# antbern/gridmap-slam-robot

Measured on AMD Instinct MI355X. Metric: particle-scan evals/sec, higher is better.
Workload: dtype f64; 1 GPU; C3: 16384 particles/GPU x 720 beams (697 hits), 2048x2048 grid @ 0.02 m, full scan step (score+normalise+resample+ray-cast+likelihood rebuild; the rebuild is dirty-tile / factor-table-only: bit-identical results, likelihoodData on demand -- the reference's own every-cell rebuild is cpu_baseline.gpu_like_for_like_ms_per_step); particles_total=16384, particles_per_gpu=16384, beams=720, maps=1, maps_total=1, parallelism=single GPU, inputs=resident in HBM

## Files before the change

### gridmap_slam_robot_amd/csrc/gms_fused_kernels.hip

```cpp
#include "gms_map_kernels.hip"
#include "gms_pf_kernels.hip"
#include "gms_slam_kernels.hip"

#ifndef GMS_APPLY_BLOCKS_RIDING
#define GMS_APPLY_BLOCKS_RIDING 512
#endif

#ifndef RCF_RAYS
#define RCF_RAYS 4
#endif

template <bool LOGNORM>
__global__ void __launch_bounds__(256)
k_norm_raycast(GridDev g, const gms_beam *__restrict__ beams, int32_t B, uint32_t *__restrict__ cnt, int32_t *__restrict__ bbox,
               int32_t nw_max, uint32_t n_ray_blocks,
               const double *__restrict__ partials, int64_t nblk_global, double *__restrict__ w, const float *__restrict__ pose,
               int32_t n, int64_t offset, PackedParticle *__restrict__ packed, double *__restrict__ cum,
               double *__restrict__ chunk_tot, int64_t nchunks, double *__restrict__ p2, PfStatsDev *__restrict__ stats,
               uint32_t n_norm_blocks, double *__restrict__ logd, uint32_t *__restrict__ cnt_pend, const int32_t *__restrict__ bbox_pend,
               uint32_t n_near_blocks, const double *__restrict__ logw_lognorm, uint32_t *__restrict__ res_ticket,
               double *__restrict__ res_pre) {
    extern __shared__ __align__(16) unsigned char smem[];
    GMS_STAMP(GMS_STAMP_ROW(2, blockIdx.x), 0);
    if (blockIdx.x >= n_ray_blocks + n_norm_blocks) {
        apply_body(g, logd, cnt_pend, bbox_pend, nullptr, blockIdx.x - n_ray_blocks - n_norm_blocks, 0,
                   gridDim.x - n_ray_blocks - n_norm_blocks);
        GMS_STAMP(GMS_STAMP_ROW(2, blockIdx.x), 15);
        return;
    }
    if (blockIdx.x < n_ray_blocks) {
        __shared__ RedLds L;
        __shared__ float s_pose[3];
        const int cols[4] = { COL_SUM, COL_XW, COL_YW, COL_TW };
        double f[4];
        if (LOGNORM) {
            fold_lognorm<4>(partials, nblk_global, cols, f, L);
        } else {
            fold_sums<4>(partials, nblk_global, cols, f, L);
        }
        if (threadIdx.x == 0) {
            s_pose[0] = (float)(f[1] / f[0]);
            s_pose[1] = (float)(f[2] / f[0]);
            s_pose[2] = (float)(f[3] / f[0]);
        }
        __syncthreads();
        GMS_STAMP(GMS_STAMP_ROW(2, blockIdx.x), 1);
        if (blockIdx.x >= n_ray_blocks - n_near_blocks)
            raycast_near_body(g, beams, B, B, nullptr, 0, cnt, bbox, blockIdx.x - (n_ray_blocks - n_near_blocks), 0, smem, s_pose);
        else
            raycast_body<false, RCF_RAYS, 4>(g, beams, B, B, nullptr, 0, nullptr, cnt, bbox, nullptr, nullptr, 0, nullptr, nw_max, blockIdx.x, 0,
                                             smem, s_pose, n_near_blocks ? 1 : 0);
    } else {
        normalize_pack_body(partials, nblk_global, w, pose, n, offset, packed, cum, chunk_tot, nchunks, p2, stats,
                            blockIdx.x - n_ray_blocks, 0, LOGNORM ? logw_lognorm : (const double *)nullptr, res_ticket, n_norm_blocks,
                            res_pre, smem);
        GMS_STAMP(GMS_STAMP_ROW(2, blockIdx.x), 14);
    }
}

__global__ void __launch_bounds__(256)
k_partials_apply(double *__restrict__ w, double *__restrict__ logw, const float *__restrict__ pose, int32_t n, int64_t offset,
                 int64_t nblk_global, double *__restrict__ partials, const double *__restrict__ part, int32_t part_nseg,
                 GridDev g, double *__restrict__ logd, uint32_t *__restrict__ cnt, const int32_t *__restrict__ bbox,
                 int32_t *__restrict__ bbox_idle, PfStatsDev *__restrict__ lognorm_stats) {
    if (blockIdx.x < (uint32_t)nblk_global)
        partials_body(w, logw, pose, n, offset, nblk_global, partials, part, part_nseg, blockIdx.x, blockIdx.y, lognorm_stats);
    else
        apply_body(g, logd, cnt, bbox, bbox_idle, blockIdx.x - (uint32_t)nblk_global, blockIdx.y, gridDim.x - (uint32_t)nblk_global);
}

__global__ void __launch_bounds__(256)
k_partials_pack_apply(double *__restrict__ w, double *__restrict__ logw, const float *__restrict__ pose, int32_t n, int64_t offset,
                      int64_t nblk_global, double *__restrict__ partials, const double *__restrict__ part, int32_t part_nseg,
                      PackedParticle *__restrict__ packed_local, uint32_t n_local_blocks,
                      GridDev g, double *__restrict__ logd, uint32_t *__restrict__ cnt, const int32_t *__restrict__ bbox,
                      int32_t *__restrict__ bbox_idle) {
    if (blockIdx.x < n_local_blocks) {
        partials_body(w, logw, pose, n, offset, nblk_global, partials, part, part_nseg, (uint32_t)(offset / GMS_BLOCK) + blockIdx.x, 0);
        pack_raw_block(w, pose, n, blockIdx.x, packed_local);
    } else {
        apply_body(g, logd, cnt, bbox, bbox_idle, blockIdx.x - n_local_blocks, 0, gridDim.x - n_local_blocks);
    }
}

__global__ void __launch_bounds__(256)
k_raycast_norm_chunks(GridDev g, const gms_beam *__restrict__ beams, int32_t B, uint32_t *__restrict__ cnt, int32_t *__restrict__ bbox,
                      int32_t nw_max, uint32_t n_ray_blocks, uint32_t n_norm_blocks,
                      const double *__restrict__ partials, int64_t nblk_global, double *__restrict__ w, const float *__restrict__ pose,
                      int32_t n, int64_t offset, const PackedParticle *__restrict__ glob_raw, int64_t n_global, int64_t nchunks,
                      double *__restrict__ cum, double *__restrict__ chunk_tot, double *__restrict__ p2,
                      PfStatsDev *__restrict__ stats, uint32_t n_chunk_blocks, double *__restrict__ logd,
                      uint32_t *__restrict__ cnt_pend, const int32_t *__restrict__ bbox_pend, uint32_t n_near_blocks) {
    extern __shared__ __align__(16) unsigned char smem[];
    if (blockIdx.x >= n_ray_blocks + n_norm_blocks + n_chunk_blocks) {
        const uint32_t first = n_ray_blocks + n_norm_blocks + n_chunk_blocks;
        apply_body(g, logd, cnt_pend, bbox_pend, nullptr, blockIdx.x - first, 0, gridDim.x - first);
        return;
    }
    if (blockIdx.x < n_ray_blocks) {
        __shared__ RedLds L;
        __shared__ float s_pose[3];
        const int cols[4] = { COL_SUM, COL_XW, COL_YW, COL_TW };
        double f[4];
        fold_sums<4>(partials, nblk_global, cols, f, L);
        if (threadIdx.x == 0) {
            s_pose[0] = (float)(f[1] / f[0]);
            s_pose[1] = (float)(f[2] / f[0]);
            s_pose[2] = (float)(f[3] / f[0]);
        }
        __syncthreads();
        if (blockIdx.x >= n_ray_blocks - n_near_blocks)
            raycast_near_body(g, beams, B, B, nullptr, 0, cnt, bbox, blockIdx.x - (n_ray_blocks - n_near_blocks), 0, smem, s_pose);
        else
            raycast_body<false, RCF_RAYS, 4>(g, beams, B, B, nullptr, 0, nullptr, cnt, bbox, nullptr, nullptr, 0, nullptr, nw_max, blockIdx.x, 0,
                                             smem, s_pose, n_near_blocks ? 1 : 0);
    } else if (blockIdx.x < n_ray_blocks + n_norm_blocks) {
        normalize_own_body(partials, nblk_global, w, pose, n, offset, glob_raw, stats, blockIdx.x - n_ray_blocks);
    } else {
        chunk_sums_raw_body(glob_raw, n_global, nchunks, cum, chunk_tot, p2, nblk_global, partials,
                            blockIdx.x - n_ray_blocks - n_norm_blocks);
    }
}

template <int KH, int SPLIT>
__global__ void __launch_bounds__(256)
k_lik_resample(GridDev g, const double *__restrict__ logd, double *__restrict__ lik, double *__restrict__ fac, int64_t fac_stride,
               const double *__restrict__ taps_g, const int32_t *__restrict__ bbox, int32_t tiles_x, int32_t tiles_y,
               const uint32_t *__restrict__ cnt_pending, uint8_t *__restrict__ tile_state, uint32_t n_res_blocks,
               const PackedParticle *__restrict__ glob, int64_t n_global, int64_t nchunks, const double *__restrict__ cum,
               const double *__restrict__ chunk_off, const double *__restrict__ r01_maps, double r01, double fraction,
               int32_t n, int64_t offset,
               float *__restrict__ pose2, float *__restrict__ cs2, double *__restrict__ w2, int32_t *__restrict__ idx_out,
               const double *__restrict__ p2, int64_t nblk_global, PfStatsDev *__restrict__ stats, int32_t raw_weights,
               int32_t *__restrict__ bbox_clear, int32_t lik_mode, const double *__restrict__ res_pre) {
    extern __shared__ __align__(16) unsigned char smem[];
    GMS_STAMP(GMS_STAMP_ROW(3, blockIdx.x), 0);
    if (blockIdx.x == 0 && threadIdx.x < 4) bbox_clear[4 * blockIdx.y + threadIdx.x] = 0;
    if (blockIdx.x < n_res_blocks)
        resample_body(glob, n_global, nchunks, cum, chunk_off, r01_maps, r01, fraction, n, offset, pose2, cs2, w2, idx_out, p2,
                      nblk_global, stats, blockIdx.x, blockIdx.y, smem, raw_weights != 0, res_pre);
    else
        likelihood_body<KH, SPLIT>(g, logd, lik, fac, fac_stride, taps_g, bbox, 1, tiles_x, tiles_y, blockIdx.x - n_res_blocks,
                                   blockIdx.y, gridDim.x - n_res_blocks, smem, cnt_pending, tile_state, lik_mode);
    GMS_STAMP(GMS_STAMP_ROW(3, blockIdx.x), blockIdx.x < n_res_blocks ? 1 : 2);
}

__global__ void __launch_bounds__(256)
k_deskew_motion(const double *__restrict__ angle, const double *__restrict__ distance, const uint8_t *__restrict__ hit, int32_t length,
// ... 160 lines not shown
```

### gridmap_slam_robot_amd/csrc/gms_map_kernels.hip

```cpp
#include "gms_device.h"

__device__ __forceinline__ void bbox_decode(const int32_t *bb, int32_t W, int32_t H, int32_t &x0, int32_t &y0,
                                            int32_t &x1, int32_t &y1) {
    x0 = W - 1 - bb[0]; y0 = H - 1 - bb[1]; x1 = bb[2]; y1 = bb[3];
}


struct RayMeta {
    int32_t x0, y0, x_inc, y_inc, n_eff, hit;
    float sx, sy, measured;
    int32_t hx, hy;
};

#define RC_VALID 0x80000000u
#define RC_BOX_MARGIN 5

typedef __attribute__((address_space(3))) uint64_t gms_lds_u64;
typedef __attribute__((address_space(3))) uint32_t gms_lds_u32;
typedef __attribute__((address_space(3))) double gms_lds_f64;
__device__ __forceinline__ uint32_t lds_offset(const uint64_t *p) { return (uint32_t)(uintptr_t)(const gms_lds_u64 *)p; }
__device__ __forceinline__ void lds_publish_u64(uint64_t *p, uint64_t v) {
    asm volatile("ds_write_b64 %0, %1" : : "v"(lds_offset(p)), "v"(v) : "memory");
}
__device__ __forceinline__ void lds_poll_2xu64(const uint64_t *p0, const uint64_t *p1, uint64_t &a, uint64_t &c) {
    asm volatile("ds_read_b64 %0, %2\n\t"
                 "ds_read_b64 %1, %3\n\t"
                 "s_waitcnt lgkmcnt(0)"
                 : "=&v"(a), "=&v"(c) : "v"(lds_offset(p0)), "v"(lds_offset(p1)) : "memory");
}

__device__ __forceinline__ RayMeta ray_meta(const GridDev &g, const RayIn &ray, RayDev &r) {
    RayMeta mt;
    ray_init(r, ray.sx + 0.5f, ray.sy + 0.5f, ray.ex + 0.5f, ray.ey + 0.5f, g.extra);
    mt.x0 = r.x; mt.y0 = r.y; mt.x_inc = r.x_inc; mt.y_inc = r.y_inc;
    mt.sx = ray.sx; mt.sy = ray.sy; mt.measured = ray.measured; mt.hit = ray.hit;
    const bool inb0 = !(r.x < 0 || r.x >= g.W || r.y < 0 || r.y >= g.H);
    mt.n_eff = (inb0 && r.n > 0) ? min(r.n, g.W + g.H + 1) : 0;
    const int64_t ax = llabs((int64_t)j_d2i(floor((double)(ray.ex + 0.5f))) - (int64_t)r.x) + g.extra + RC_BOX_MARGIN;
    const int64_t ay = llabs((int64_t)j_d2i(floor((double)(ray.ey + 0.5f))) - (int64_t)r.y) + g.extra + RC_BOX_MARGIN;
    const int32_t moves = mt.n_eff > 0 ? mt.n_eff - 1 : 0;
    mt.hx = min(max(r.x + r.x_inc * (int32_t)min((int64_t)moves, ax), 0), g.W - 1);
    mt.hy = min(max(r.y + r.y_inc * (int32_t)min((int64_t)moves, ay), 0), g.H - 1);
    return mt;
}
__device__ __forceinline__ void ray_box(const GridDev &g, const RayMeta &mt, int32_t bb[4]) {
    if (mt.n_eff <= 0) { bb[0] = bb[1] = bb[2] = bb[3] = 0; return; }
    bb[0] = g.W - 1 - min(mt.x0, mt.hx); bb[1] = g.H - 1 - min(mt.y0, mt.hy);
    bb[2] = max(mt.x0, mt.hx) + 1;       bb[3] = max(mt.y0, mt.hy) + 1;
}
__device__ __forceinline__ void bbox_raise_wave(int32_t bb[4], int32_t lane, int32_t *__restrict__ bbox_map) {
#define GMS_STEP_(O) { _Pragma("unroll") for (int q = 0; q < 4; q++) bb[q] = max(bb[q], wave_xor<O>(bb[q])); }
    GMS_BUTTERFLY(GMS_STEP_)
#undef GMS_STEP_
    if (lane == 0 && bb[2] > 0)
        for (int q = 0; q < 4; q++) atomicMax(&bbox_map[q], bb[q]);
}

struct RayWalk {
    float err, ndx, dy;
    uint32_t ycount;
};
__device__ __forceinline__ RayWalk ray_walk_begin(const RayDev &r) {
    RayWalk k;
    k.err = r.error; k.ndx = -r.dx; k.dy = r.dy; k.ycount = 0;
    asm volatile("" : "+v"(k.ndx), "+v"(k.dy));
    return k;
}
__device__ __forceinline__ void ray_phase_a(RayWalk &k, int32_t w0, int32_t w1, uint64_t *__restrict__ slots, int32_t stride, int32_t slot) {
    float err = k.err;
    const float ndx = k.ndx, dy = k.dy;
    uint32_t ycount = k.ycount;
    for (int32_t w = w0; w < w1; ++w) {
        uint32_t word = 0;
        float t;
#define GMS_DDA_STEP "v_cmp_lt_f32_e32 vcc, 0, %0\n\tv_cndmask_b32_e32 %2, %3, %4, vcc\n\tv_add_f32_e32 %0, %0, %2\n\tv_addc_co_u32_e32 %1, vcc, %1, %1, vcc\n\t"
// ... 37 lines not shown
        const int32_t ny = (int32_t)(((uint32_t)(sl >> 32) & ~RC_VALID) + __popc((uint32_t)sl & ((1u << j) - 1u)));
        const int32_t nx = k - ny;
        const int32_t cx = mt.x0 + mt.x_inc * nx, cy = mt.y0 + mt.y_inc * ny;
        valid = !(cx < 0 || cx >= g.W || cy < 0 || cy >= g.H);
        if (valid) {
            const float d = cell_distance(mt.sx, mt.sy, cx, cy);
            const int32_t cls = sensor_class(d, mt.measured, mt.hit, g.half_tol);
            if (TRACE) {
                if (k < cap) {
                    const size_t o = (size_t)b * cap + k;
                    if (t_cells) { t_cells[2 * o] = cx; t_cells[2 * o + 1] = cy; }
                    if (t_cls) t_cls[o] = (uint8_t)cls;
                }
            } else if (cls != 1) {
                const uint32_t inc = cls == 0 ? 1u : 0x10000u;
                const uint32_t ux = (uint32_t)(cx - tile.x0), uy = (uint32_t)(cy - tile.y0);
                if (ux < (uint32_t)tile.w && uy < (uint32_t)tile.h) {
                    const uint32_t ci = uy * (uint32_t)tile.w + ux;
                    __hip_atomic_fetch_add((gms_lds_u32 *)(tile.cells) + (ci >> 1), (cls == 0 ? 1u : 0x100u) << ((ci & 1u) << 4),
                                           __ATOMIC_RELAXED, __HIP_MEMORY_SCOPE_WORKGROUP);
                } else {
                    atomicAdd(&mcnt[(size_t)cy * g.W + cx], inc);
                    if (__builtin_expect(cx < min(mt.x0, mt.hx) || cx > max(mt.x0, mt.hx) || cy < min(mt.y0, mt.hy) || cy > max(mt.y0, mt.hy), 0)) {
                        atomicMax(&bbox_map[0], g.W - 1 - cx); atomicMax(&bbox_map[1], g.H - 1 - cy);
                        atomicMax(&bbox_map[2], cx + 1);       atomicMax(&bbox_map[3], cy + 1);
                    }
                }
            }
        }
    }
    return __popcll(__ballot(valid));
}

template <bool TRACE, int RC_RAYS, int NWAVES = RC_RAYS>
__device__ __forceinline__ void
raycast_body(const GridDev &g, const gms_beam *__restrict__ beams, int32_t B, int32_t beam_stride,
             const float *__restrict__ poses, int32_t pose_stride, const RayIn *__restrict__ single,
             uint32_t *__restrict__ cnt, int32_t *__restrict__ bbox, int32_t *__restrict__ t_cells,
             uint8_t *__restrict__ t_cls, int32_t cap, int32_t *__restrict__ t_counts, int32_t nw_max,
             uint32_t bx, uint32_t by, unsigned char *smem, const float *pose_lds, int32_t first_blk = 0) {
    uint64_t *s_slots = reinterpret_cast<uint64_t *>(smem);
    __shared__ RayMeta s_meta[RC_RAYS];
    __shared__ int32_t s_count[RC_RAYS];

    const int32_t mi = (int32_t)by;
    const int32_t lane = threadIdx.x & 63;
    const int32_t wave = __builtin_amdgcn_readfirstlane(threadIdx.x >> 6);
    for (int32_t i = threadIdx.x; i < nw_max * RC_RAYS; i += NWAVES * 64) s_slots[i] = 0ull;
    RayDev r;
    r.dx = r.dy = r.error = 0.0f; r.x = r.y = r.x_inc = r.y_inc = r.n = 0;
    int32_t my_n_eff = 0;
    if (wave == 0 && lane < RC_RAYS) {
        const int32_t b = (int32_t)bx * RC_RAYS + lane;
        RayMeta mt;
        mt.n_eff = 0; mt.x0 = mt.y0 = mt.x_inc = mt.y_inc = mt.hit = 0; mt.sx = mt.sy = mt.measured = 0.0f;
        if (b < B) {
            RayIn ray;
            if (single) ray = *single;
            else ray = make_ray(g, beams[(size_t)mi * beam_stride + b], pose_lds ? pose_lds : poses + (size_t)pose_stride * mi);
            mt = ray_meta(g, ray, r);
        }
        my_n_eff = mt.n_eff;
        s_meta[lane] = mt;
        s_count[lane] = 0;
    }
    __syncthreads();
    GMS_STAMP(GMS_STAMP_ROW(2, blockIdx.x), 2);
    if (!TRACE && first_blk == 0 && wave == (NWAVES > 1 ? 1 : 0)) {
        int32_t hb[4] = { 0, 0, 0, 0 };
        if (lane < RC_RAYS) ray_box(g, s_meta[lane], hb);
        bbox_raise_wave(hb, lane, bbox + 4 * mi);
    }
    if (wave == 0) {
        if (lane < RC_RAYS) {
            RayWalk wk = ray_walk_begin(r);
            ray_phase_a(wk, 0, (my_n_eff + 31) >> 5, s_slots, RC_RAYS, lane);
        }
        GMS_STAMP(GMS_STAMP_ROW(2, blockIdx.x), 3);
    } else {
        int32_t nblk_max = 0;
#pragma unroll
        for (int q = 0; q < RC_RAYS; q++) nblk_max = max(nblk_max, (s_meta[q].n_eff + 63) >> 6);
        constexpr int32_t NC = NWAVES - 1;
        for (int32_t q = wave - 1 + first_blk * RC_RAYS; q < nblk_max * RC_RAYS; q += NC) {
            const int32_t blk = q / RC_RAYS, ray = q - blk * RC_RAYS;
            const RayMeta mt = s_meta[ray];
            if (blk * 64 >= mt.n_eff) continue;
            const int32_t n = ray_phase_b<TRACE>(g, mt, s_slots, RC_RAYS, ray, blk, lane, TRACE ? nullptr : cnt + (size_t)mi * g.cells, TRACE ? nullptr : bbox + 4 * mi,
                                                 (int32_t)bx * RC_RAYS + ray, t_cells, t_cls, cap);
            if (TRACE && lane == 0) atomicAdd(&s_count[ray], n);
        }
        GMS_STAMP_T(64, GMS_STAMP_ROW(2, blockIdx.x), 4);
    }
    if (TRACE) {
        __syncthreads();
        const int32_t b = (int32_t)bx * RC_RAYS + (int32_t)threadIdx.x;
        if (threadIdx.x < RC_RAYS && b < B && t_counts) t_counts[b] = s_count[threadIdx.x];
    } else {
        GMS_STAMP(GMS_STAMP_ROW(2, blockIdx.x), 5);
    }
}

#ifndef RCN_RAYS
#define RCN_RAYS 16
#endif
#define RCN_TILE_CELLS 12288
#define RCN_LDS_BYTES (2 * RCN_RAYS * 8 + RCN_TILE_CELLS * 2)
static_assert(RCN_RAYS >= 1 && RCN_RAYS <= 64, "the near-field producer is one wavefront, a lane per ray");

__device__ __forceinline__ void
raycast_near_body(const GridDev &g, const gms_beam *__restrict__ beams, int32_t B, int32_t beam_stride,
                  const float *__restrict__ poses, int32_t pose_stride, uint32_t *__restrict__ cnt, int32_t *__restrict__ bbox,
                  uint32_t bx, uint32_t by, unsigned char *smem, const float *pose_lds) {
    uint64_t *s_slots = reinterpret_cast<uint64_t *>(smem);
    uint32_t *s_tile = reinterpret_cast<uint32_t *>(s_slots + 2 * RCN_RAYS);
    __shared__ RayMeta s_nmeta[RCN_RAYS];
    __shared__ int32_t s_nbox[4];
    const int32_t mi = (int32_t)by;
    const int32_t lane = threadIdx.x & 63;
    const int32_t wave = __builtin_amdgcn_readfirstlane(threadIdx.x >> 6);
    const int32_t nwaves = __builtin_amdgcn_readfirstlane((int32_t)(blockDim.x >> 6));
    for (int32_t i = threadIdx.x; i < 2 * RCN_RAYS; i += blockDim.x) s_slots[i] = 0ull;
    RayDev r;
    r.dx = r.dy = r.error = 0.0f; r.x = r.y = r.x_inc = r.y_inc = r.n = 0;
    int32_t my_nwords = 0;
    if (wave == 0) {
        const int32_t b = (int32_t)bx * RCN_RAYS + lane;
        RayMeta mt;
        mt.n_eff = 0; mt.x0 = mt.y0 = mt.x_inc = mt.y_inc = mt.hit = 0; mt.sx = mt.sy = mt.measured = 0.0f;
        int32_t bx0 = INT32_MAX, by0 = INT32_MAX, bx1 = INT32_MIN, by1 = INT32_MIN;
        if (lane < RCN_RAYS && b < B) {
            const RayIn ray = make_ray(g, beams[(size_t)mi * beam_stride + b], pose_lds ? pose_lds : poses + (size_t)pose_stride * mi);
            mt = ray_meta(g, ray, r);
            if (mt.n_eff > 0) {
                const int32_t steps = min(mt.n_eff, 64) - 1;
                const float tot = r.dx + r.dy;
                const int32_t mx = tot > 0.0f ? min(steps, (int32_t)((float)steps * (r.dx / tot)) + 2) : 0;
                const int32_t my = tot > 0.0f ? min(steps, (int32_t)((float)steps * (r.dy / tot)) + 2) : 0;
                const int32_t ex = mt.x0 + mt.x_inc * mx, ey = mt.y0 + mt.y_inc * my;
                bx0 = max(min(mt.x0, ex), 0); bx1 = min(max(mt.x0, ex), g.W - 1);
                by0 = max(min(mt.y0, ey), 0); by1 = min(max(mt.y0, ey), g.H - 1);
            }
        }
        my_nwords = min((mt.n_eff + 31) >> 5, 2);
        if (lane < RCN_RAYS) s_nmeta[lane] = mt;
#define GMS_STEP_(O) { bx0 = min(bx0, wave_xor<O>(bx0)); by0 = min(by0, wave_xor<O>(by0)); bx1 = max(bx1, wave_xor<O>(bx1)); by1 = max(by1, wave_xor<O>(by1)); }
        GMS_BUTTERFLY(GMS_STEP_)
#undef GMS_STEP_
        if (lane == 0) { s_nbox[0] = bx0; s_nbox[1] = by0; s_nbox[2] = bx1; s_nbox[3] = by1; }
    }
    __syncthreads();
    CountTile tile;
    tile.cells = s_tile; tile.x0 = s_nbox[0]; tile.y0 = s_nbox[1];
    tile.w = s_nbox[2] >= s_nbox[0] ? s_nbox[2] - s_nbox[0] + 1 : 0;
    tile.h = s_nbox[3] >= s_nbox[1] ? s_nbox[3] - s_nbox[1] + 1 : 0;
    if ((int64_t)tile.w * tile.h > RCN_TILE_CELLS || RCN_RAYS * (1 + g.extra) > 255) tile.w = tile.h = 0;
    const int32_t tcells = tile.w * tile.h;
    for (int32_t i = threadIdx.x; i < (tcells + 1) / 2; i += blockDim.x) s_tile[i] = 0u;
    __syncthreads();
    GMS_STAMP(GMS_STAMP_ROW(2, blockIdx.x), 9);
    if (wave == 0) {
        RayWalk wk = ray_walk_begin(r);
        if (lane < RCN_RAYS && my_nwords > 0) ray_phase_a(wk, 0, my_nwords, s_slots, RCN_RAYS, lane);
    } else {
        if (wave == 1) {
            int32_t hb[4] = { 0, 0, 0, 0 };
            if (lane < RCN_RAYS) ray_box(g, s_nmeta[lane], hb);
            bbox_raise_wave(hb, lane, bbox + 4 * mi);
        }
        for (int32_t ray = wave - 1; ray < RCN_RAYS; ray += nwaves - 1) {
            RayMeta mt = s_nmeta[ray];
            if (mt.n_eff <= 0) continue;
            mt.n_eff = min(mt.n_eff, 64);
            ray_phase_b<false>(g, mt, s_slots, RCN_RAYS, ray, 0, lane, cnt + (size_t)mi * g.cells, bbox + 4 * mi, 0, nullptr, nullptr, 0, tile, 0);
        }
    }
    __syncthreads();
    GMS_STAMP(GMS_STAMP_ROW(2, blockIdx.x), 10);
    uint32_t *mcnt = cnt + (size_t)mi * g.cells;
    for (int32_t ry = wave; ry < tile.h; ry += nwaves) {
        const int32_t cy = tile.y0 + ry, rbase = ry * tile.w;
        for (int32_t rx = lane; rx < tile.w; rx += 64) {
            const int32_t i = rbase + rx;
            const uint32_t v = (s_tile[i >> 1] >> ((i & 1) << 4)) & 0xffffu;
            if (v) atomicAdd(&mcnt[(size_t)cy * g.W + tile.x0 + rx], (v & 0xffu) | ((v >> 8) << 16));
        }
    }
    GMS_STAMP(GMS_STAMP_ROW(2, blockIdx.x), 11);
}
#define GMS_RAYCAST_NEAR_MIN_BEAMS 512
static inline uint32_t rc_near_blocks(const gms_map *m, int32_t B) {
    if (!m->raycast_near || B < (m->raycast_near == 2 ? 32 : GMS_RAYCAST_NEAR_MIN_BEAMS)) return 0u;
    return (uint32_t)((B + RCN_RAYS - 1) / RCN_RAYS);
}

template <bool TRACE, int RC_RAYS>
__global__ void __launch_bounds__(RC_RAYS * 64)
k_raycast(GridDev g, const gms_beam *__restrict__ beams, int32_t B, int32_t beam_stride,
          const float *__restrict__ poses, int32_t pose_stride, const RayIn *__restrict__ single,
          uint32_t *__restrict__ cnt, int32_t *__restrict__ bbox, int32_t *__restrict__ t_cells,
          uint8_t *__restrict__ t_cls, int32_t cap, int32_t *__restrict__ t_counts, int32_t nw_max, uint32_t n_near_blocks) {
    extern __shared__ __align__(16) unsigned char smem[];
    if (!TRACE && RC_RAYS == 4 && n_near_blocks && blockIdx.x >= gridDim.x - n_near_blocks) {
        raycast_near_body(g, beams, B, beam_stride, poses, pose_stride, cnt, bbox, blockIdx.x - (gridDim.x - n_near_blocks), blockIdx.y, smem,
                          nullptr);
        return;
    }
    raycast_body<TRACE, RC_RAYS>(g, beams, B, beam_stride, poses, pose_stride, single, cnt, bbox, t_cells, t_cls, cap, t_counts,
                                 nw_max, blockIdx.x, blockIdx.y, smem, nullptr, n_near_blocks ? 1 : 0);
}

#define RCT_RAYS 64
#define RCT_THREADS 1024
#define RCT_WORDS 16
#define RCT_TILE_CELLS 32768
#define RCT_LDS_BYTES (RCT_WORDS * RCT_RAYS * 8 + RCT_TILE_CELLS * 2)

__device__ void apply_slices(const GridDev &g, double *__restrict__ logd, uint32_t *__restrict__ cnt, const int32_t *__restrict__ bbox,
                             uint32_t first_block);

__global__ void __launch_bounds__(RCT_THREADS)
k_raycast_tile(GridDev g, const gms_beam *__restrict__ beams, int32_t B, int32_t beam_stride, const float *__restrict__ poses,
               int32_t pose_stride, uint32_t *__restrict__ cnt, int32_t *__restrict__ bbox, uint32_t n_ray_blocks,
               double *__restrict__ logd, uint32_t *__restrict__ cnt_pend, const int32_t *__restrict__ bbox_pend) {
    extern __shared__ __align__(16) unsigned char smem[];
    if (blockIdx.x >= n_ray_blocks) {
        apply_slices(g, logd, cnt_pend, bbox_pend, n_ray_blocks);
        return;
    }
    uint64_t *s_slots = reinterpret_cast<uint64_t *>(smem);
    uint32_t *s_tile = reinterpret_cast<uint32_t *>(s_slots + RCT_WORDS * RCT_RAYS);
    __shared__ RayMeta s_meta[RCT_RAYS];
    __shared__ int32_t s_box[5];

    const int32_t mi = blockIdx.y;
    const int32_t lane = threadIdx.x & 63;
    const int32_t wave = __builtin_amdgcn_readfirstlane(threadIdx.x >> 6);
    RayDev r;
    r.dx = r.dy = r.error = 0.0f; r.x = r.y = r.x_inc = r.y_inc = r.n = 0;
    int32_t my_nwords = 0;
    if (wave == 0) {
        const int32_t b = (int32_t)blockIdx.x * RCT_RAYS + lane;
// ... 460 lines not shown
                    for (int32_t i = 0; i < ntaps; i++) total += taps_s[i] * hs[(r + i) * PHS + c];
                    if (wr_lik) mlik[(size_t)gy * g.W + gx] = total;
                    if (wr_fac) FAC_STORE(&mfac[(size_t)gy * g.fpitch + gx], lik_factor(g, total));
                }
            }
        }
    }
    if (g.tile_stats && threadIdx.x == 0) {
        uint32_t *row = g.tile_stats + 4 * (bx & 63u);
        if (ts_left) atomicAdd(row + 0, ts_left);
        if (ts_const_kept) atomicAdd(row + 1, ts_const_kept);
        if (ts_const_written) atomicAdd(row + 2, ts_const_written);
        if (ts_blurred) atomicAdd(row + 3, ts_blurred);
    }
}

template <int KH, bool PENDING, int SPLIT = 1>
__global__ void __launch_bounds__(256) GMS_LIK_WAVES
k_likelihood(GridDev g, const double *__restrict__ logd, double *__restrict__ lik, double *__restrict__ fac,
             int64_t fac_stride, const double *__restrict__ taps_g, const int32_t *__restrict__ bbox, int32_t dirty_only,
             int32_t tiles_x, int32_t tiles_y, uint8_t *__restrict__ tile_state, const uint32_t *__restrict__ cnt_pending,
             int32_t *__restrict__ bbox_clear, int32_t mode) {
    extern __shared__ __align__(16) unsigned char smem[];
    if (bbox_clear && blockIdx.x == 0 && threadIdx.x < 4) bbox_clear[4 * blockIdx.y + threadIdx.x] = 0;
    likelihood_body<KH, SPLIT>(g, logd, lik, fac, fac_stride, taps_g, bbox, dirty_only, tiles_x, tiles_y, blockIdx.x, blockIdx.y,
                               gridDim.x, smem, PENDING ? cnt_pending : (const uint32_t *)nullptr, tile_state, mode);
}

__global__ void __launch_bounds__(256)
k_raycast_apply(GridDev g, const gms_beam *__restrict__ beams, int32_t B, int32_t beam_stride, const float *__restrict__ poses,
                int32_t pose_stride, uint32_t *__restrict__ cnt, int32_t *__restrict__ bbox_next, int32_t nw_max, uint32_t n_ray_blocks,
                uint32_t n_near_blocks, double *__restrict__ logd, uint32_t *__restrict__ cnt_pend, const int32_t *__restrict__ bbox_pend) {
    extern __shared__ __align__(16) unsigned char smem[];
    if (blockIdx.x < n_ray_blocks)
        raycast_body<false, 4>(g, beams, B, beam_stride, poses, pose_stride, nullptr, cnt, bbox_next, nullptr, nullptr, 0, nullptr, nw_max,
                               blockIdx.x, 0, smem, nullptr, n_near_blocks ? 1 : 0);
    else if (blockIdx.x < n_ray_blocks + n_near_blocks)
        raycast_near_body(g, beams, B, beam_stride, poses, pose_stride, cnt, bbox_next, blockIdx.x - n_ray_blocks, 0, smem, nullptr);
    else
        apply_body(g, logd, cnt_pend, bbox_pend, nullptr, blockIdx.x - n_ray_blocks - n_near_blocks, 0, gridDim.x - n_ray_blocks - n_near_blocks);
}

__global__ void k_factors(GridDev g, const double *__restrict__ lik, double *__restrict__ fac, int64_t fac_stride) {
    const int32_t mi = blockIdx.y;
    double *mfac = fac + (size_t)mi * fac_stride;
    for (int64_t i = (int64_t)blockIdx.x * blockDim.x + threadIdx.x; i < fac_stride; i += (int64_t)gridDim.x * blockDim.x) {
        const int32_t gy = (int32_t)(i / g.fpitch), gx = (int32_t)(i - (int64_t)gy * g.fpitch);
        mfac[i] = gx < g.W && gy < g.H ? lik_factor(g, lik[(size_t)mi * g.cells + (size_t)gy * g.W + gx]) : 1.0;
    }
}

__device__ __forceinline__ void combine_body(const double *__restrict__ logs, int32_t n_maps, int64_t cells, double *__restrict__ out) {
    for (int64_t i = (int64_t)blockIdx.x * blockDim.x + threadIdx.x; i < cells; i += (int64_t)gridDim.x * blockDim.x) {
        double product = 1.0;
        for (int32_t m = 0; m < n_maps; m++) {
            const double l = logs[(size_t)m * cells + i];
            product *= 1.0 - ((double)1.0f - (double)1.0f / (1.0 + exp(l)));
        }
        const double odds = 1.0 - product;
        out[i] = log(odds / ((double)1.0f - odds));
    }
}
__global__ void k_combine(const double *__restrict__ logs, int32_t n_maps, int64_t cells, double *__restrict__ out) { combine_body(logs, n_maps, cells, out); }

__device__ __forceinline__ void deskew_body(const double *__restrict__ angle, const double *__restrict__ distance,
                                            const uint8_t *__restrict__ hit, int32_t length, double d_center, double d_theta,
                                            gms_beam *__restrict__ out, int32_t i) {
    if (i >= length) return;
    const double d_i = -(double)(length - i) / (double)length;
    const double delta_theta = d_theta * d_i, delta_x = d_center * d_i;
    const double a = angle[i] + delta_theta;
    const double x_a = distance[i] * cos(a) + delta_x;
    const double y_a = distance[i] * sin(a);
// ... 422 lines not shown
```

Before: 372.6 million particle-scan evals/s.

## Replicate ray setup per wavefront and drop LDS metadata barriers in raycast

Every wavefront now computes the ray walk initialisation itself instead of one producer wave writing RayMeta into shared memory. Consumer waves fetch a given ray's metadata with readlane from their own registers, which removes the s_meta/s_nmeta LDS arrays and two block barriers. Beam loads and LDS slot and tile clears move into a prologue that runs before the pose reduction, so they overlap with the fold. The near-field tile bounds are computed redundantly per wave with butterfly reductions. The cost is duplicated per-ray arithmetic in every wave and higher register pressure.

```diff
diff --git a/gridmap_slam_robot_amd/csrc/gms_fused_kernels.hip b/gridmap_slam_robot_amd/csrc/gms_fused_kernels.hip
--- a/gridmap_slam_robot_amd/csrc/gms_fused_kernels.hip
+++ b/gridmap_slam_robot_amd/csrc/gms_fused_kernels.hip
@@ -30,7 +30,9 @@
     }
     if (blockIdx.x < n_ray_blocks) {
         __shared__ RedLds L;
-        __shared__ float s_pose[3];
+        const bool near = blockIdx.x >= n_ray_blocks - n_near_blocks;
+        const RayPre pre = near ? raycast_near_prologue(beams, B, B, blockIdx.x - (n_ray_blocks - n_near_blocks), 0, smem)
+                                : raycast_prologue<RCF_RAYS, 4>(beams, B, B, nullptr, nw_max, blockIdx.x, 0, smem);
         const int cols[4] = { COL_SUM, COL_XW, COL_YW, COL_TW };
         double f[4];
         if (LOGNORM) {
@@ -38,18 +40,10 @@
         } else {
             fold_sums<4>(partials, nblk_global, cols, f, L);
         }
-        if (threadIdx.x == 0) {
-            s_pose[0] = (float)(f[1] / f[0]);
-            s_pose[1] = (float)(f[2] / f[0]);
-            s_pose[2] = (float)(f[3] / f[0]);
-        }
-        __syncthreads();
+        const float wpose[3] = { (float)(f[1] / f[0]), (float)(f[2] / f[0]), (float)(f[3] / f[0]) };
         GMS_STAMP(GMS_STAMP_ROW(2, blockIdx.x), 1);
-        if (blockIdx.x >= n_ray_blocks - n_near_blocks)
-            raycast_near_body(g, beams, B, B, nullptr, 0, cnt, bbox, blockIdx.x - (n_ray_blocks - n_near_blocks), 0, smem, s_pose);
-        else
-            raycast_body<false, RCF_RAYS, 4>(g, beams, B, B, nullptr, 0, nullptr, cnt, bbox, nullptr, nullptr, 0, nullptr, nw_max, blockIdx.x, 0,
-                                             smem, s_pose, n_near_blocks ? 1 : 0);
+        if (near) raycast_near_body(g, pre, wpose, cnt, bbox, 0, smem);
+        else raycast_body<false, RCF_RAYS, 4>(g, pre, wpose, B, nullptr, cnt, bbox, nullptr, nullptr, 0, nullptr, blockIdx.x, 0, smem, n_near_blocks ? 1 : 0);
     } else {
         normalize_pack_body(partials, nblk_global, w, pose, n, offset, packed, cum, chunk_tot, nchunks, p2, stats,
                             blockIdx.x - n_ray_blocks, 0, LOGNORM ? logw_lognorm : (const double *)nullptr, res_ticket, n_norm_blocks,
@@ -99,21 +93,15 @@
     }
     if (blockIdx.x < n_ray_blocks) {
         __shared__ RedLds L;
-        __shared__ float s_pose[3];
+        const bool near = blockIdx.x >= n_ray_blocks - n_near_blocks;
+        const RayPre pre = near ? raycast_near_prologue(beams, B, B, blockIdx.x - (n_ray_blocks - n_near_blocks), 0, smem)
+                                : raycast_prologue<RCF_RAYS, 4>(beams, B, B, nullptr, nw_max, blockIdx.x, 0, smem);
         const int cols[4] = { COL_SUM, COL_XW, COL_YW, COL_TW };
         double f[4];
         fold_sums<4>(partials, nblk_global, cols, f, L);
-        if (threadIdx.x == 0) {
-            s_pose[0] = (float)(f[1] / f[0]);
-            s_pose[1] = (float)(f[2] / f[0]);
-            s_pose[2] = (float)(f[3] / f[0]);
-        }
-        __syncthreads();
-        if (blockIdx.x >= n_ray_blocks - n_near_blocks)
-            raycast_near_body(g, beams, B, B, nullptr, 0, cnt, bbox, blockIdx.x - (n_ray_blocks - n_near_blocks), 0, smem, s_pose);
-        else
-            raycast_body<false, RCF_RAYS, 4>(g, beams, B, B, nullptr, 0, nullptr, cnt, bbox, nullptr, nullptr, 0, nullptr, nw_max, blockIdx.x, 0,
-                                             smem, s_pose, n_near_blocks ? 1 : 0);
+        const float wpose[3] = { (float)(f[1] / f[0]), (float)(f[2] / f[0]), (float)(f[3] / f[0]) };
+        if (near) raycast_near_body(g, pre, wpose, cnt, bbox, 0, smem);
+        else raycast_body<false, RCF_RAYS, 4>(g, pre, wpose, B, nullptr, cnt, bbox, nullptr, nullptr, 0, nullptr, blockIdx.x, 0, smem, n_near_blocks ? 1 : 0);
     } else if (blockIdx.x < n_ray_blocks + n_norm_blocks) {
         normalize_own_body(partials, nblk_global, w, pose, n, offset, glob_raw, stats, blockIdx.x - n_ray_blocks);
     } else {
diff --git a/gridmap_slam_robot_amd/csrc/gms_map_kernels.hip b/gridmap_slam_robot_amd/csrc/gms_map_kernels.hip
--- a/gridmap_slam_robot_amd/csrc/gms_map_kernels.hip
+++ b/gridmap_slam_robot_amd/csrc/gms_map_kernels.hip
@@ -29,18 +29,40 @@
                  : "=&v"(a), "=&v"(c) : "v"(lds_offset(p0)), "v"(lds_offset(p1)) : "memory");
 }
 
-__device__ __forceinline__ RayMeta ray_meta(const GridDev &g, const RayIn &ray, RayDev &r) {
+__device__ __forceinline__ int32_t ray_walk_init(const GridDev &g, const RayIn &ray, RayDev &r) {
+    ray_init(r, ray.sx + 0.5f, ray.sy + 0.5f, ray.ex + 0.5f, ray.ey + 0.5f, g.extra);
+    const bool inb0 = !(r.x < 0 || r.x >= g.W || r.y < 0 || r.y >= g.H);
+    return (inb0 && r.n > 0) ? min(r.n, g.W + g.H + 1) : 0;
+}
+__device__ __forceinline__ RayMeta ray_meta_rest(const GridDev &g, const RayIn &ray, const RayDev &r, int32_t n_eff) {
     RayMeta mt;
-    ray_init(r, ray.sx + 0.5f, ray.sy + 0.5f, ray.ex + 0.5f, ray.ey + 0.5f, g.extra);
     mt.x0 = r.x; mt.y0 = r.y; mt.x_inc = r.x_inc; mt.y_inc = r.y_inc;
     mt.sx = ray.sx; mt.sy = ray.sy; mt.measured = ray.measured; mt.hit = ray.hit;
-    const bool inb0 = !(r.x < 0 || r.x >= g.W || r.y < 0 || r.y >= g.H);
-    mt.n_eff = (inb0 && r.n > 0) ? min(r.n, g.W + g.H + 1) : 0;
+    mt.n_eff = n_eff;
     const int64_t ax = llabs((int64_t)j_d2i(floor((double)(ray.ex + 0.5f))) - (int64_t)r.x) + g.extra + RC_BOX_MARGIN;
     const int64_t ay = llabs((int64_t)j_d2i(floor((double)(ray.ey + 0.5f))) - (int64_t)r.y) + g.extra + RC_BOX_MARGIN;
     const int32_t moves = mt.n_eff > 0 ? mt.n_eff - 1 : 0;
     mt.hx = min(max(r.x + r.x_inc * (int32_t)min((int64_t)moves, ax), 0), g.W - 1);
     mt.hy = min(max(r.y + r.y_inc * (int32_t)min((int64_t)moves, ay), 0), g.H - 1);
+    return mt;
+}
+__device__ __forceinline__ RayMeta ray_meta(const GridDev &g, const RayIn &ray, RayDev &r) {
+    const int32_t n_eff = ray_walk_init(g, ray, r);
+    return ray_meta_rest(g, ray, r, n_eff);
+}
+__device__ __forceinline__ RayMeta ray_meta_of_lane(const RayMeta &m, int32_t l) {
+    RayMeta o;
+#define GMS_RL_(F) o.F = __builtin_amdgcn_readlane(m.F, l)
+#define GMS_RLF_(F) o.F = __int_as_float(__builtin_amdgcn_readlane(__float_as_int(m.F), l))
+    GMS_RL_(x0); GMS_RL_(y0); GMS_RL_(x_inc); GMS_RL_(y_inc); GMS_RL_(n_eff); GMS_RL_(hit); GMS_RL_(hx); GMS_RL_(hy);
+    GMS_RLF_(sx); GMS_RLF_(sy); GMS_RLF_(measured);
+#undef GMS_RL_
+#undef GMS_RLF_
+    return o;
+}
+__device__ __forceinline__ RayMeta ray_meta_none() {
+    RayMeta mt;
+    mt.n_eff = 0; mt.x0 = mt.y0 = mt.x_inc = mt.y_inc = mt.hit = mt.hx = mt.hy = 0; mt.sx = mt.sy = mt.measured = 0.0f;
     return mt;
 }
 __device__ __forceinline__ void ray_box(const GridDev &g, const RayMeta &mt, int32_t bb[4]) {
@@ -144,63 +166,82 @@
     return __popcll(__ballot(valid));
 }
 
+struct RayPre {
+    gms_beam beam;
+    bool in;
+};
+template <int RC_RAYS, int NWAVES>
+__device__ __forceinline__ RayPre
+raycast_prologue(const gms_beam *__restrict__ beams, int32_t B, int32_t beam_stride, const RayIn *__restrict__ single,
+                 int32_t nw_max, uint32_t bx, uint32_t by, unsigned char *smem) {
+    uint64_t *s_slots = reinterpret_cast<uint64_t *>(smem);
+    const int32_t lane = threadIdx.x & 63;
+    const int32_t b = (int32_t)bx * RC_RAYS + lane;
+    RayPre pre;
+    pre.in = lane < RC_RAYS && b < B;
+    pre.beam.local_x = pre.beam.local_y = pre.beam.distance = 0.0; pre.beam.hit = 0;
+    if (pre.in && !single) {
+        const gms_beam *src = beams + (size_t)by * beam_stride + b;
+        pre.beam.local_x = src->local_x; pre.beam.local_y = src->local_y; pre.beam.distance = src->distance; pre.beam.hit = src->hit;
+    }
+    for (int32_t i = threadIdx.x; i < nw_max * RC_RAYS; i += NWAVES * 64) s_slots[i] = 0ull;
+    return pre;
+}
+
 template <bool TRACE, int RC_RAYS, int NWAVES = RC_RAYS>
 __device__ __forceinline__ void
-raycast_body(const GridDev &g, const gms_beam *__restrict__ beams, int32_t B, int32_t beam_stride,
-             const float *__restrict__ poses, int32_t pose_stride, const RayIn *__restrict__ single,
+raycast_body(const GridDev &g, const RayPre &pre, const float (&pose)[3], int32_t B, const RayIn *__restrict__ single,
              uint32_t *__restrict__ cnt, int32_t *__restrict__ bbox, int32_t *__restrict__ t_cells,
-             uint8_t *__restrict__ t_cls, int32_t cap, int32_t *__restrict__ t_counts, int32_t nw_max,
-             uint32_t bx, uint32_t by, unsigned char *smem, const float *pose_lds, int32_t first_blk = 0) {
+             uint8_t *__restrict__ t_cls, int32_t cap, int32_t *__restrict__ t_counts,
+             uint32_t bx, uint32_t by, unsigned char *smem, int32_t first_blk = 0) {
+    static_assert(NWAVES >= 2 && RC_RAYS <= 64, "one producer wavefront (a lane per ray) and at least one consumer");
     uint64_t *s_slots = reinterpret_cast<uint64_t *>(smem);
-    __shared__ RayMeta s_meta[RC_RAYS];
     __shared__ int32_t s_count[RC_RAYS];
 
     const int32_t mi = (int32_t)by;
     const int32_t lane = threadIdx.x & 63;
     const int32_t wave = __builtin_amdgcn_readfirstlane(threadIdx.x >> 6);
-    for (int32_t i = threadIdx.x; i < nw_max * RC_RAYS; i += NWAVES * 64) s_slots[i] = 0ull;
     RayDev r;
     r.dx = r.dy = r.error = 0.0f; r.x = r.y = r.x_inc = r.y_inc = r.n = 0;
+    RayIn ray;
+    ray.sx = ray.sy = ray.ex = ray.ey = ray.measured = 0.0f; ray.hit = 0;
     int32_t my_n_eff = 0;
-    if (wave == 0 && lane < RC_RAYS) {
-        const int32_t b = (int32_t)bx * RC_RAYS + lane;
-        RayMeta mt;
-        mt.n_eff = 0; mt.x0 = mt.y0 = mt.x_inc = mt.y_inc = mt.hit = 0; mt.sx = mt.sy = mt.measured = 0.0f;
-        if (b < B) {
-            RayIn ray;
-            if (single) ray = *single;
-            else ray = make_ray(g, beams[(size_t)mi * beam_stride + b], pose_lds ? pose_lds : poses + (size_t)pose_stride * mi);
-            mt = ray_meta(g, ray, r);
-        }
-        my_n_eff = mt.n_eff;
-        s_meta[lane] = mt;
-        s_count[lane] = 0;
-    }
-    __syncthreads();
-    GMS_STAMP(GMS_STAMP_ROW(2, blockIdx.x), 2);
-    if (!TRACE && first_blk == 0 && wave == (NWAVES > 1 ? 1 : 0)) {
-        int32_t hb[4] = { 0, 0, 0, 0 };
-        if (lane < RC_RAYS) ray_box(g, s_meta[lane], hb);
-        bbox_raise_wave(hb, lane, bbox + 4 * mi);
+    if (pre.in) {
+        if (single) ray = *single;
+        else ray = make_ray(g, pre.beam, pose);
+        my_n_eff = ray_walk_init(g, ray, r);
+    }
+    if (TRACE) {
+        if (threadIdx.x < RC_RAYS) s_count[threadIdx.x] = 0;
+        __syncthreads();
     }
     if (wave == 0) {
+        GMS_STAMP(GMS_STAMP_ROW(2, blockIdx.x), 2);
         if (lane < RC_RAYS) {
             RayWalk wk = ray_walk_begin(r);
             ray_phase_a(wk, 0, (my_n_eff + 31) >> 5, s_slots, RC_RAYS, lane);
         }
         GMS_STAMP(GMS_STAMP_ROW(2, blockIdx.x), 3);
     } else {
-        int32_t nblk_max = 0;
-#pragma unroll
-        for (int q = 0; q < RC_RAYS; q++) nblk_max = max(nblk_max, (s_meta[q].n_eff + 63) >> 6);
+        const RayMeta mine = pre.in ? ray_meta_rest(g, ray, r, my_n_eff) : ray_meta_none();
+        if (!TRACE && first_blk == 0 && wave == 1) {
+            int32_t hb[4];
+            ray_box(g, mine, hb);
+            bbox_raise_wave(hb, lane, bbox + 4 * mi);
+        }
+        int32_t nblk_max = (mine.n_eff + 63) >> 6;
+#define GMS_STEP_(O) nblk_max = max(nblk_max, wave_xor<O>(nblk_max));
+        GMS_BUTTERFLY(GMS_STEP_)
+#undef GMS_STEP_
+        nblk_max = __builtin_amdgcn_readfirstlane(nblk_max);
         constexpr int32_t NC = NWAVES - 1;
         for (int32_t q = wave - 1 + first_blk * RC_RAYS; q < nblk_max * RC_RAYS; q += NC) {
-            const int32_t blk = q / RC_RAYS, ray = q - blk * RC_RAYS;
-            const RayMeta mt = s_meta[ray];
+            const int32_t blk = q / RC_RAYS, rq = q - blk * RC_RAYS;
+            const RayMeta mt = ray_meta_of_lane(mine, rq);
             if (blk * 64 >= mt.n_eff) continue;
-            const int32_t n = ray_phase_b<TRACE>(g, mt, s_slots, RC_RAYS, ray, blk, lane, TRACE ? nullptr : cnt + (size_t)mi * g.cells, TRACE ? nullptr : bbox + 4 * mi,
-                                                 (int32_t)bx * RC_RAYS + ray, t_cells, t_cls, cap);
-            if (TRACE && lane == 0) atomicAdd(&s_count[ray], n);
+            const int32_t n = ray_phase_b<TRACE>(g, mt, s_slots, RC_RAYS, rq, blk, lane, TRACE ? nullptr : cnt + (size_t)mi * g.cells, TRACE ? nullptr : bbox + 4 * mi,
+                                                 (int32_t)bx * RC_RAYS + rq, t_cells, t_cls, cap);
+            if (TRACE && lane == 0) atomicAdd(&s_count[rq], n);
         }
         GMS_STAMP_T(64, GMS_STAMP_ROW(2, blockIdx.x), 4);
     }
@@ -220,71 +261,88 @@
 #define RCN_LDS_BYTES (2 * RCN_RAYS * 8 + RCN_TILE_CELLS * 2)
 static_assert(RCN_RAYS >= 1 && RCN_RAYS <= 64, "the near-field producer is one wavefront, a lane per ray");
 
+__device__ __forceinline__ RayPre
+raycast_near_prologue(const gms_beam *__restrict__ beams, int32_t B, int32_t beam_stride, uint32_t bx, uint32_t by, unsigned char *smem) {
+    uint64_t *s_slots = reinterpret_cast<uint64_t *>(smem);
+    uint4 *s_tile4 = reinterpret_cast<uint4 *>(s_slots + 2 * RCN_RAYS);
+    static_assert((2 * RCN_RAYS * 8) % 16 == 0 && RCN_TILE_CELLS % 8 == 0, "the tile is cleared in 16-byte stores");
+    const int32_t lane = threadIdx.x & 63;
+    const int32_t b = (int32_t)bx * RCN_RAYS + lane;
+    RayPre pre;
+    pre.in = lane < RCN_RAYS && b < B;
+    pre.beam.local_x = pre.beam.local_y = pre.beam.distance = 0.0; pre.beam.hit = 0;
+    if (pre.in) {
+        const gms_beam *src = beams + (size_t)by * beam_stride + b;
+        pre.beam.local_x = src->local_x; pre.beam.local_y = src->local_y; pre.beam.distance = src->distance; pre.beam.hit = src->hit;
+    }
+    for (int32_t i = threadIdx.x; i < 2 * RCN_RAYS; i += blockDim.x) s_slots[i] = 0ull;
+    for (int32_t i = threadIdx.x; i < RCN_TILE_CELLS / 8; i += blockDim.x) s_tile4[i] = make_uint4(0u, 0u, 0u, 0u);
+    return pre;
+}
+
+__device__ __forceinline__ CountTile
+near_tile(const GridDev &g, const RayDev &r, int32_t n_eff, uint32_t *s_tile) {
+    int32_t bx0 = INT32_MAX, by0 = INT32_MAX, bx1 = INT32_MIN, by1 = INT32_MIN;
+    if (n_eff > 0) {
+        const int32_t steps = min(n_eff, 64) - 1;
+        const float tot = r.dx + r.dy;
+        const int32_t mx = tot > 0.0f ? min(steps, (int32_t)((float)steps * (r.dx / tot)) + 2) : 0;
+        const int32_t my = tot > 0.0f ? min(steps, (int32_t)((float)steps * (r.dy / tot)) + 2) : 0;
+        const int32_t ex = r.x + r.x_inc * mx, ey = r.y + r.y_inc * my;
+        bx0 = max(min(r.x, ex), 0); bx1 = min(max(r.x, ex), g.W - 1);
+        by0 = max(min(r.y, ey), 0); by1 = min(max(r.y, ey), g.H - 1);
+    }
+#define GMS_STEP_(O) { bx0 = min(bx0, wave_xor<O>(bx0)); by0 = min(by0, wave_xor<O>(by0)); bx1 = max(bx1, wave_xor<O>(bx1)); by1 = max(by1, wave_xor<O>(by1)); }
+    GMS_BUTTERFLY(GMS_STEP_)
+#undef GMS_STEP_
+    bx0 = __builtin_amdgcn_readfirstlane(bx0); by0 = __builtin_amdgcn_readfirstlane(by0);
+    bx1 = __builtin_amdgcn_readfirstlane(bx1); by1 = __builtin_amdgcn_readfirstlane(by1);
+    CountTile tile;
+    tile.cells = s_tile; tile.x0 = bx0; tile.y0 = by0;
+    tile.w = bx1 >= bx0 ? bx1 - bx0 + 1 : 0;
+    tile.h = by1 >= by0 ? by1 - by0 + 1 : 0;
+    if ((int64_t)tile.w * tile.h > RCN_TILE_CELLS || RCN_RAYS * (1 + g.extra) > 255) tile.w = tile.h = 0;
+    return tile;
+}
+
 __device__ __forceinline__ void
-raycast_near_body(const GridDev &g, const gms_beam *__restrict__ beams, int32_t B, int32_t beam_stride,
-                  const float *__restrict__ poses, int32_t pose_stride, uint32_t *__restrict__ cnt, int32_t *__restrict__ bbox,
-                  uint32_t bx, uint32_t by, unsigned char *smem, const float *pose_lds) {
+raycast_near_body(const GridDev &g, const RayPre &pre, const float (&pose)[3], uint32_t *__restrict__ cnt, int32_t *__restrict__ bbox,
+                  uint32_t by, unsigned char *smem) {
     uint64_t *s_slots = reinterpret_cast<uint64_t *>(smem);
     uint32_t *s_tile = reinterpret_cast<uint32_t *>(s_slots + 2 * RCN_RAYS);
-    __shared__ RayMeta s_nmeta[RCN_RAYS];
-    __shared__ int32_t s_nbox[4];
     const int32_t mi = (int32_t)by;
     const int32_t lane = threadIdx.x & 63;
     const int32_t wave = __builtin_amdgcn_readfirstlane(threadIdx.x >> 6);
     const int32_t nwaves = __builtin_amdgcn_readfirstlane((int32_t)(blockDim.x >> 6));
-    for (int32_t i = threadIdx.x; i < 2 * RCN_RAYS; i += blockDim.x) s_slots[i] = 0ull;
     RayDev r;
     r.dx = r.dy = r.error = 0.0f; r.x = r.y = r.x_inc = r.y_inc = r.n = 0;
-    int32_t my_nwords = 0;
+    RayIn ray;
+    ray.sx = ray.sy = ray.ex = ray.ey = ray.measured = 0.0f; ray.hit = 0;
+    int32_t my_n_eff = 0;
+    if (pre.in) {
+        ray = make_ray(g, pre.beam, pose);
+        my_n_eff = ray_walk_init(g, ray, r);
+    }
+    CountTile tile;
     if (wave == 0) {
-        const int32_t b = (int32_t)bx * RCN_RAYS + lane;
-        RayMeta mt;
-        mt.n_eff = 0; mt.x0 = mt.y0 = mt.x_inc = mt.y_inc = mt.hit = 0; mt.sx = mt.sy = mt.measured = 0.0f;
-        int32_t bx0 = INT32_MAX, by0 = INT32_MAX, bx1 = INT32_MIN, by1 = INT32_MIN;
-        if (lane < RCN_RAYS && b < B) {
-            const RayIn ray = make_ray(g, beams[(size_t)mi * beam_stride + b], pose_lds ? pose_lds : poses + (size_t)pose_stride * mi);
-            mt = ray_meta(g, ray, r);
-            if (mt.n_eff > 0) {
-                const int32_t steps = min(mt.n_eff, 64) - 1;
-                const float tot = r.dx + r.dy;
-                const int32_t mx = tot > 0.0f ? min(steps, (int32_t)((float)steps * (r.dx / tot)) + 2) : 0;
-                const int32_t my = tot > 0.0f ? min(steps, (int32_t)((float)steps * (r.dy / tot)) + 2) : 0;
-                const int32_t ex = mt.x0 + mt.x_inc * mx, ey = mt.y0 + mt.y_inc * my;
-                bx0 = max(min(mt.x0, ex), 0); bx1 = min(max(mt.x0, ex), g.W - 1);
-                by0 = max(min(mt.y0, ey), 0); by1 = min(max(mt.y0, ey), g.H - 1);
-            }
-        }
-        my_nwords = min((mt.n_eff + 31) >> 5, 2);
-        if (lane < RCN_RAYS) s_nmeta[lane] = mt;
-#define GMS_STEP_(O) { bx0 = min(bx0, wave_xor<O>(bx0)); by0 = min(by0, wave_xor<O>(by0)); bx1 = max(bx1, wave_xor<O>(bx1)); by1 = max(by1, wave_xor<O>(by1)); }
-        GMS_BUTTERFLY(GMS_STEP_)
-#undef GMS_STEP_
-        if (lane == 0) { s_nbox[0] = bx0; s_nbox[1] = by0; s_nbox[2] = bx1; s_nbox[3] = by1; }
-    }
-    __syncthreads();
-    CountTile tile;
-    tile.cells = s_tile; tile.x0 = s_nbox[0]; tile.y0 = s_nbox[1];
-    tile.w = s_nbox[2] >= s_nbox[0] ? s_nbox[2] - s_nbox[0] + 1 : 0;
-    tile.h = s_nbox[3] >= s_nbox[1] ? s_nbox[3] - s_nbox[1] + 1 : 0;
-    if ((int64_t)tile.w * tile.h > RCN_TILE_CELLS || RCN_RAYS * (1 + g.extra) > 255) tile.w = tile.h = 0;
-    const int32_t tcells = tile.w * tile.h;
-    for (int32_t i = threadIdx.x; i < (tcells + 1) / 2; i += blockDim.x) s_tile[i] = 0u;
-    __syncthreads();
-    GMS_STAMP(GMS_STAMP_ROW(2, blockIdx.x), 9);
-    if (wave == 0) {
+        GMS_STAMP(GMS_STAMP_ROW(2, blockIdx.x), 9);
+        const int32_t my_nwords = min((my_n_eff + 31) >> 5, 2);
         RayWalk wk = ray_walk_begin(r);
         if (lane < RCN_RAYS && my_nwords > 0) ray_phase_a(wk, 0, my_nwords, s_slots, RCN_RAYS, lane);
+        tile = near_tile(g, r, my_n_eff, s_tile);
     } else {
+        const RayMeta mine = pre.in ? ray_meta_rest(g, ray, r, my_n_eff) : ray_meta_none();
+        tile = near_tile(g, r, my_n_eff, s_tile);
         if (wave == 1) {
-            int32_t hb[4] = { 0, 0, 0, 0 };
-            if (lane < RCN_RAYS) ray_box(g, s_nmeta[lane], hb);
+            int32_t hb[4];
+            ray_box(g, mine, hb);
             bbox_raise_wave(hb, lane, bbox + 4 * mi);
         }
-        for (int32_t ray = wave - 1; ray < RCN_RAYS; ray += nwaves - 1) {
-            RayMeta mt = s_nmeta[ray];
+        for (int32_t rq = wave - 1; rq < RCN_RAYS; rq += nwaves - 1) {
+            RayMeta mt = ray_meta_of_lane(mine, rq);
             if (mt.n_eff <= 0) continue;
             mt.n_eff = min(mt.n_eff, 64);
-            ray_phase_b<false>(g, mt, s_slots, RCN_RAYS, ray, 0, lane, cnt + (size_t)mi * g.cells, bbox + 4 * mi, 0, nullptr, nullptr, 0, tile, 0);
+            ray_phase_b<false>(g, mt, s_slots, RCN_RAYS, rq, 0, lane, cnt + (size_t)mi * g.cells, bbox + 4 * mi, 0, nullptr, nullptr, 0, tile, 0);
         }
     }
     __syncthreads();
@@ -313,13 +371,15 @@
           uint32_t *__restrict__ cnt, int32_t *__restrict__ bbox, int32_t *__restrict__ t_cells,
           uint8_t *__restrict__ t_cls, int32_t cap, int32_t *__restrict__ t_counts, int32_t nw_max, uint32_t n_near_blocks) {
     extern __shared__ __align__(16) unsigned char smem[];
-    if (!TRACE && RC_RAYS == 4 && n_near_blocks && blockIdx.x >= gridDim.x - n_near_blocks) {
-        raycast_near_body(g, beams, B, beam_stride, poses, pose_stride, cnt, bbox, blockIdx.x - (gridDim.x - n_near_blocks), blockIdx.y, smem,
-                          nullptr);
-        return;
-    }
-    raycast_body<TRACE, RC_RAYS>(g, beams, B, beam_stride, poses, pose_stride, single, cnt, bbox, t_cells, t_cls, cap, t_counts,
-                                 nw_max, blockIdx.x, blockIdx.y, smem, nullptr, n_near_blocks ? 1 : 0);
+    const bool near = !TRACE && RC_RAYS == 4 && n_near_blocks && blockIdx.x >= gridDim.x - n_near_blocks;
+    const RayPre pre = near ? raycast_near_prologue(beams, B, beam_stride, blockIdx.x - (gridDim.x - n_near_blocks), blockIdx.y, smem)
+                            : raycast_prologue<RC_RAYS, RC_RAYS>(beams, B, beam_stride, single, nw_max, blockIdx.x, blockIdx.y, smem);
+    float pose[3] = { 0.0f, 0.0f, 0.0f };
+    if (!single) { const float *p = poses + (size_t)pose_stride * blockIdx.y; pose[0] = p[0]; pose[1] = p[1]; pose[2] = p[2]; }
+    __syncthreads();
+    if (near) { raycast_near_body(g, pre, pose, cnt, bbox, blockIdx.y, smem); return; }
+    raycast_body<TRACE, RC_RAYS>(g, pre, pose, B, single, cnt, bbox, t_cells, t_cls, cap, t_counts, blockIdx.x, blockIdx.y, smem,
+                                 n_near_blocks ? 1 : 0);
 }
 
 #define RCT_RAYS 64
@@ -846,13 +906,17 @@
                 int32_t pose_stride, uint32_t *__restrict__ cnt, int32_t *__restrict__ bbox_next, int32_t nw_max, uint32_t n_ray_blocks,
                 uint32_t n_near_blocks, double *__restrict__ logd, uint32_t *__restrict__ cnt_pend, const int32_t *__restrict__ bbox_pend) {
     extern __shared__ __align__(16) unsigned char smem[];
-    if (blockIdx.x < n_ray_blocks)
-        raycast_body<false, 4>(g, beams, B, beam_stride, poses, pose_stride, nullptr, cnt, bbox_next, nullptr, nullptr, 0, nullptr, nw_max,
-                               blockIdx.x, 0, smem, nullptr, n_near_blocks ? 1 : 0);
-    else if (blockIdx.x < n_ray_blocks + n_near_blocks)
-        raycast_near_body(g, beams, B, beam_stride, poses, pose_stride, cnt, bbox_next, blockIdx.x - n_ray_blocks, 0, smem, nullptr);
-    else
+    if (blockIdx.x >= n_ray_blocks + n_near_blocks) {
         apply_body(g, logd, cnt_pend, bbox_pend, nullptr, blockIdx.x - n_ray_blocks - n_near_blocks, 0, gridDim.x - n_ray_blocks - n_near_blocks);
+        return;
+    }
+    const bool near = blockIdx.x >= n_ray_blocks;
+    const RayPre pre = near ? raycast_near_prologue(beams, B, beam_stride, blockIdx.x - n_ray_blocks, 0, smem)
+                            : raycast_prologue<4, 4>(beams, B, beam_stride, nullptr, nw_max, blockIdx.x, 0, smem);
+    const float pose[3] = { poses[0], poses[1], poses[2] };
+    __syncthreads();
+    if (near) raycast_near_body(g, pre, pose, cnt, bbox_next, 0, smem);
+    else raycast_body<false, 4>(g, pre, pose, B, nullptr, cnt, bbox_next, nullptr, nullptr, 0, nullptr, blockIdx.x, 0, smem, n_near_blocks ? 1 : 0);
 }
 
 __global__ void k_factors(GridDev g, const double *__restrict__ lik, double *__restrict__ fac, int64_t fac_stride) {
```

Result: faster. 378.0 million particle-scan evals/s (median of 6 runs) (+1.4%).
